# mhamilton723/STEGO

Measured on NVIDIA H100. Metric: train-step images/sec, higher is better.
Workload: dtype bf16

## Files before the change

include/stego_b200.h:

```cpp
#ifndef STEGO_B200_H_
#define STEGO_B200_H_

#ifdef __cplusplus
extern "C" {
#endif

#define STEGO_API

STEGO_API int stego_version(void);
STEGO_API const char* stego_last_error(void);
STEGO_API long long stego_launch_count(void);

STEGO_API int stego_gemm_bf16(const void* A, int lda, int a_mn_major, const void* B, int ldb, int b_mn_major,
                              int M, int N, int K, void* out, int ldo, int out_bf16, const float* bias, int act,
                              const float* residual, int ldr, int row_div, int splits, int atomic_out,
                              void* stream);

STEGO_API int stego_gemm_bf16_batched(const void* A, int lda, long long a_batch_stride, int a_mn_major, const void* B,
                                      int ldb, long long b_batch_stride, int b_mn_major, int batch, int M, int N, int K,
                                      void* out, int ldo, long long out_batch_stride, int out_bf16, const float* bias,
                                      int act, void* stream);

STEGO_API int stego_vit_patchify(const float* img, void* out_bf16, int B, int H, int W, int patch, void* stream);
STEGO_API int stego_vit_patchify_bf16(const void* img_bf16, void* out_bf16, int B, int H, int W, int patch,
                                      void* stream);
STEGO_API int stego_vit_patchify_tta(const void* img, int img_is_bf16, void* out_bf16, int B, int H, int W, int patch,
                                     void* stream);
STEGO_API int stego_vit_cls_rows(float* x, const float* cls_token, const float* pos_embed, int B, int ntok, int E,
                                 void* stream);
STEGO_API int stego_layernorm_bf16(const float* x, const float* gamma, const float* beta, void* out_bf16, int rows,
                                   int E, float eps, int drop_cls_ntok, void* stream);
STEGO_API int stego_layernorm_gap(const float* x, const float* gamma, const float* beta, float* out, int B, int ntok,
                                  int E, float eps, void* stream);
STEGO_API int stego_linear_rows_f32(const float* x, const void* w_bf16, int ldw, const float* bias, float* out, int B,
                                    int N, int K, void* stream);
STEGO_API int stego_attention_fwd(const void* qkv, void* out, int B, int N, int E, int heads, void* stream);
STEGO_API int stego_attention_probs(const void* qkv, float* probs, int B, int N, int E, int heads, void* stream);

STEGO_API int stego_sample_norm_fwd(const void* src, const void* src_pos, int src_is_bf16, long long stride_b,
                                    long long stride_c, long long stride_y, long long stride_x,
                                    const float* chan_scale, const float* chan_scale_pos, const float* coords1,
                                    const float* coords2, const long long* perms, void* tiles, int B, int C,
                                    int Cpad, int H, int W, int feature_samples, int nslots, int perms_are_raw_randperm,
                                    void* stream);
STEGO_API int stego_sample_labels_fwd(const void* label, const void* label_pos, int label_bytes, const float* coords1,
                                      const float* coords2, const long long* perms, void* tiles, int B, int n_classes,
                                      int Cpad, int H, int W, int feature_samples, int nslots,
                                      int perms_are_raw_randperm, void* stream);
STEGO_API int stego_corr_loss_fwd(const void* feat_tiles, const void* code_tiles, int B, int feature_samples, int E,
                                  int D, int nslots, int ncalls, const int* slot_of_call_host,
                                  const float* shifts_host, int pointwise, int zero_clamp, int stabilize,
                                  float* partials, float* stats, float* cd_out, float* fdc_out, float* loss_out,
                                  void* stream);
STEGO_API int stego_corr_loss_bwd(const void* feat_tiles, const void* code_tiles, int B, int feature_samples, int E,
                                  int D, int nslots, int ncalls, const int* slot_of_call_host,
                                  const float* shifts_host, int pointwise, int zero_clamp, int stabilize,
                                  const float* stats, const float* gscale, const float* gelem, const float* gcd,
                                  float* dtiles, void* stream);
STEGO_API int stego_sample_norm_bwd(const float* code, const float* code_pos, long long stride_b, long long stride_c,
                                    long long stride_y, long long stride_x, const float* coords1,
                                    const float* coords2, const long long* perms, const float* dtiles, float* dcode,
                                    float* dcode_pos, int B, int C, int H, int W, int feature_samples, int nslots,
                                    int perms_are_raw_randperm, void* stream);

STEGO_API int stego_corr_loss_tiled_fwd(const void* feat_tiles, const void* code_tiles, int B, int feature_samples,
                                        int E, int D, int nslots, int ncalls, const int* slot_of_call_host,
                                        const float* shifts_host, int pointwise, int zero_clamp, int stabilize,
                                        float* row_partials, float* row_means, float* stats, float* cd_out,
                                        float* fdc_out, float* loss_out, void* stream);
STEGO_API int stego_corr_loss_tiled_bwd(const void* feat_tiles, const void* code_tiles, int B, int feature_samples,
                                        int E, int D, int nslots, int ncalls, const int* slot_of_call_host,
                                        const float* shifts_host, int pointwise, int zero_clamp, int stabilize,
                                        const float* stats, const float* row_means, const float* gscale,
                                        const float* gelem, const float* gcd, float* dtiles, void* stream);

STEGO_API int stego_salience_counts(const void* salience, const void* salience_pos, int mask_bytes, int B, int H, int W,
                                    int* counts, void* stream);
STEGO_API int stego_salience_coords(const void* salience, const void* salience_pos, int mask_bytes, int B, int H, int W,
                                    int feature_samples, long long seed, const long long* offsets,
                                    const void* draws_u32, const float* u_reg1, const float* u_reg2,
                                    const float* u_keep, float* coords1, float* coords2, void* scratch, void* stream);
STEGO_API long long stego_salience_scratch_bytes(int B, int H, int W);

STEGO_API int stego_aug_record_words(void);
STEGO_API long long stego_aug_scratch_bytes(int B, int size);
STEGO_API int stego_aug_views(const float* img, long long stride_b, long long stride_c, long long stride_y,
                              long long stride_x, int B, int H, int W, int size, const int* records, void* scratch,
                              float* img_aug, float* coord_aug, void* stream);

STEGO_API int stego_tb_tables(double* edges, float* thresholds);
STEGO_API int stego_tb_histogram(const float* values, long long n, const float* thresholds, long long* counts,
                                 double* cta_partials, double* stats, void* stream);
STEGO_API int stego_corr_loss_fwd_hist(const void* feat_tiles, const void* code_tiles, int B, int feature_samples,
                                       int E, int D, int nslots, int ncalls, const int* slot_of_call_host,
                                       const float* shifts_host, int pointwise, int zero_clamp, int stabilize,
                                       float* partials, float* stats, float* cd_out, float* fdc_out, float* loss_out,
                                       const float* thresholds, long long* hist_counts, double* hist_cta_partials,
                                       double* hist_stats, void* stream);
STEGO_API int stego_corr_loss_tiled_fwd_hist(const void* feat_tiles, const void* code_tiles, int B,
// ... 189 lines not shown
```

stego_b200/csrc/attention.cu:

```cuda
#include <stdlib.h>

#include "common.cuh"
#include "host_util.h"

namespace stego {

constexpr int ATT_BQ = 128;
constexpr int ATT_BKV = 64;
constexpr int ATT_D = 64;
constexpr int ATT_STAGES = 4;
constexpr int ATT_THREADS = 288;

constexpr uint32_t ATT_Q_BYTES = 128 * 64 * 2;
constexpr uint32_t ATT_KV_BYTES = 64 * 64 * 2;
constexpr uint32_t ATT_SMEM_Q = 0;
constexpr uint32_t ATT_SMEM_KV = ATT_Q_BYTES;
constexpr uint32_t ATT_SMEM_BAR = ATT_SMEM_KV + ATT_STAGES * 2 * ATT_KV_BYTES;
constexpr uint32_t ATT_SMEM_TOTAL = ATT_SMEM_BAR + 128;

struct AttnParams {
  int N;
  int E;
  float scale_log2e;
};

__global__ void __launch_bounds__(ATT_THREADS, 2)
attention_fwd_kernel(const __grid_constant__ CUtensorMap tmQKV, const __grid_constant__ CUtensorMap tmOut, AttnParams p) {
  extern __shared__ __align__(1024) uint8_t smem[];
  if ((smem_u32(smem) & 1023u) != 0u) __trap();
  uint64_t* bars = reinterpret_cast<uint64_t*>(smem + ATT_SMEM_BAR);
  uint64_t* q_full = bars;
  uint64_t* kv_full = bars + 1;
  uint64_t* kv_empty = kv_full + ATT_STAGES;

  const int warp = threadIdx.x >> 5;
  const int lane = threadIdx.x & 31;
  const int q0 = blockIdx.x * ATT_BQ;
  const int head = blockIdx.y;
  const int img = blockIdx.z;
  const int nkv = (p.N + ATT_BKV - 1) / ATT_BKV;

  if (threadIdx.x == 0) {
    mbar_init(q_full, 1);
    for (int s = 0; s < ATT_STAGES; ++s) {
      mbar_init(&kv_full[s], 1);
      mbar_init(&kv_empty[s], 2);
    }
    fence_barrier_init();
  }
  __syncthreads();

  if (warp == 8) {
    if (lane == 0) {
      tma_prefetch_desc(&tmQKV);
      tma_prefetch_desc(&tmOut);
      mbar_arrive_expect_tx(q_full, ATT_Q_BYTES);
      tma_load_3d(smem + ATT_SMEM_Q, &tmQKV, q_full, head * ATT_D, q0, img);
      tma_load_3d(smem + ATT_SMEM_Q + ATT_Q_BYTES / 2, &tmQKV, q_full, head * ATT_D, q0 + 64, img);
      uint32_t stage = 0, phase = 0;
      for (int j = 0; j < nkv; ++j) {
        mbar_wait(&kv_empty[stage], phase ^ 1u);
        uint8_t* sk = smem + ATT_SMEM_KV + stage * 2 * ATT_KV_BYTES;
        mbar_arrive_expect_tx(&kv_full[stage], 2 * ATT_KV_BYTES);
        tma_load_3d(sk, &tmQKV, &kv_full[stage], p.E + head * ATT_D, j * ATT_BKV, img);
        tma_load_3d(sk + ATT_KV_BYTES, &tmQKV, &kv_full[stage], 2 * p.E + head * ATT_D, j * ATT_BKV, img);
        if (++stage == ATT_STAGES) { stage = 0; phase ^= 1u; }
      }
    }
    return;
  }

  const int wg = warp >> 2;
  const int wq = warp & 3;
  const bool leader = (threadIdx.x & 127) == 0;
  const float c = p.scale_log2e;
  constexpr uint32_t DESC_HI = smem_desc_hi_sw128(1024);
  uint8_t* sq = smem + ATT_SMEM_Q + wg * (ATT_Q_BYTES / 2);
  const uint32_t q_lo = smem_desc_lo(smem_u32(sq), 16);
  const uint32_t k_lo0 = smem_desc_lo(smem_u32(smem + ATT_SMEM_KV), 16);
  const uint32_t v_lo0 = smem_desc_lo(smem_u32(smem + ATT_SMEM_KV + ATT_KV_BYTES), 8192);
  float o[32];
#pragma unroll
  for (int i = 0; i < 32; ++i) o[i] = 0.f;
  float m_run[2] = {-INFINITY, -INFINITY}, l_run[2] = {0.f, 0.f};
  mbar_wait(q_full, 0);
  uint32_t stage = 0, phase = 0;
  for (int j = 0; j < nkv; ++j) {
    mbar_wait(&kv_full[stage], phase);
    const uint32_t k_lo = k_lo0 + stage * ((2 * ATT_KV_BYTES) >> 4);
    const uint32_t v_lo = v_lo0 + stage * ((2 * ATT_KV_BYTES) >> 4);
    float s[32];
    wgmma_fence();
#pragma unroll
    for (uint32_t k = 0; k < ATT_D / 16; ++k)
      wgmma_ss<64, 0, 0>(s, smem_desc_join(q_lo + k * 2, DESC_HI), smem_desc_join(k_lo + k * 2, DESC_HI), k > 0 ? 1u : 0u);
    wgmma_commit();
    wgmma_wait<0>();
    fence_operands(s);
    const int valid = p.N - j * ATT_BKV;
    if (valid < ATT_BKV) {
#pragma unroll
      for (int i = 0; i < 32; ++i)
        if (8 * (i >> 2) + 2 * (lane & 3) + (i & 1) >= valid) s[i] = -INFINITY;
    }
    float alpha[2], mc[2];
#pragma unroll
    for (int h = 0; h < 2; ++h) {
      float mx = -INFINITY;
#pragma unroll
      for (int i = 0; i < 8; ++i) mx = fmaxf(mx, fmaxf(s[4 * i + 2 * h], s[4 * i + 2 * h + 1]));
      mx = fmaxf(mx, __shfl_xor_sync(0xffffffffu, mx, 1));
      mx = fmaxf(mx, __shfl_xor_sync(0xffffffffu, mx, 2));
      const float m_new = fmaxf(m_run[h], mx);
      alpha[h] = ex2_approx((m_run[h] - m_new) * c);
      m_run[h] = m_new;
      mc[h] = m_new * c;
    }
    uint32_t a[4][4];
    float rs[2] = {0.f, 0.f};
#pragma unroll
    for (int i = 0; i < 8; ++i) {
#pragma unroll
// ... 244 lines not shown
```

stego_b200/csrc/gemm.cu:

```cuda
#include <stdlib.h>
#include <string.h>

#include "common.cuh"
#include "epilogue.cuh"
#include "host_util.h"

namespace stego {

constexpr int GEMM_BM = 128;
constexpr int GEMM_BN = 128;
constexpr int GEMM_BK = 64;
constexpr int GEMM_THREADS = 384;
constexpr uint32_t GEMM_STAGE_BYTES = (GEMM_BM + GEMM_BN) * GEMM_BK * 2;
constexpr uint32_t GEMM_CHUNK_BYTES = GEMM_BM * 128;

struct GemmParams {
  int M, N, K;
  int splits;
  int kb_per_split;
  void* out;
  int ldo;
  int out_bf16;
  const float* bias;
  int act;
  const float* residual;
  int ldr;
  int row_div;
  int atomic;
  int vec_ok;
  int reduce_add;
  int batch;
  long long out_bs;
  long long res_bs;
};

template <int BN>
__device__ __forceinline__ void gemm_bias_act(float (&acc)[BN / 2], const GemmParams& p, int col_base) {
  if (p.bias != nullptr) {
#pragma unroll
    for (int c = 0; c < BN / 8; ++c) {
      const int col = col_base + 8 * c;
      float b0 = 0.f, b1 = 0.f;
      if (col + 1 < p.N && p.vec_ok) {
        const float2 b2 = __ldg(reinterpret_cast<const float2*>(p.bias + col));
        b0 = b2.x; b1 = b2.y;
      } else {
        if (col < p.N) b0 = __ldg(p.bias + col);
        if (col + 1 < p.N) b1 = __ldg(p.bias + col + 1);
      }
      acc[4 * c + 0] += b0; acc[4 * c + 1] += b1;
      acc[4 * c + 2] += b0; acc[4 * c + 3] += b1;
    }
  }
  if (p.act == 1) {
    if (p.out_bf16) {
#pragma unroll
      for (int j = 0; j < BN / 2; j += 8) gelu_erf_poly8(acc + j);
    } else {
#pragma unroll
      for (int j = 0; j < BN / 2; ++j) acc[j] = gelu_erf(acc[j]);
    }
  } else if (p.act == 2) {
#pragma unroll
    for (int j = 0; j < BN / 2; ++j) acc[j] = fmaxf(acc[j], 0.0f);
  }
}

template <int BN>
__device__ __forceinline__ void gemm_store_regs(const float (&acc)[BN / 2], const GemmParams& p, int row_top,
                                                int col_base, int tb) {
  void* const outp = p.out_bf16 ? static_cast<void*>(reinterpret_cast<bf16*>(p.out) + tb * p.out_bs)
                                : static_cast<void*>(reinterpret_cast<float*>(p.out) + tb * p.out_bs);
  const float* const resp = p.residual ? p.residual + tb * p.res_bs : nullptr;
#pragma unroll
  for (int h = 0; h < 2; ++h) {
    const int row = row_top + 8 * h;
    if (row >= p.M) continue;
    int out_row = row, res_row = row;
    if (p.row_div > 0) {
      out_row = row + row / p.row_div + 1;
      res_row = row % p.row_div + 1;
    }
    const size_t obase = static_cast<size_t>(out_row) * p.ldo;
    const size_t rbase = static_cast<size_t>(res_row) * p.ldr;
#pragma unroll
    for (int c = 0; c < BN / 8; ++c) {
      const int col = col_base + 8 * c;
      if (col >= p.N) break;
      const bool two = col + 1 < p.N;
      float x0 = acc[4 * c + 2 * h], x1 = acc[4 * c + 2 * h + 1];
      if (p.atomic) {
        float* o = reinterpret_cast<float*>(outp) + obase + col;
        atomicAdd(o, x0);
        if (two) atomicAdd(o + 1, x1);
        continue;
      }
      const bool vec = two && p.vec_ok;
      if (resp != nullptr) {
        if (vec) {
          const float2 r = *reinterpret_cast<const float2*>(resp + rbase + col);
          x0 += r.x; x1 += r.y;
        } else {
          x0 += resp[rbase + col];
          if (two) x1 += resp[rbase + col + 1];
        }
      }
      if (p.out_bf16) {
        bf16* o = reinterpret_cast<bf16*>(outp) + obase + col;
        if (vec) {
          *reinterpret_cast<uint32_t*>(o) = pack_bf16x2(x0, x1);
        } else {
          o[0] = __float2bfloat16_rn(x0);
          if (two) o[1] = __float2bfloat16_rn(x1);
        }
      } else {
        float* o = reinterpret_cast<float*>(outp) + obase + col;
// ... 27 lines not shown
    for (int h = 0; h < 2; ++h) {
#pragma unroll
      for (int e2 = 0; e2 < 2; ++e2) {
        const uint32_t rp = rbase + (64 * h + 8 * e2) * 128u;
        if constexpr (kBf16) {
#pragma unroll
          for (int j = 0; j < 8; ++j) {
            const int c = 8 * ch + j;
            st_shared_b32(rp + (((uint32_t)j ^ swz) << 4) + 4 * q,
                          pack_bf16x2(acc[h][4 * c + 2 * e2], acc[h][4 * c + 2 * e2 + 1]));
          }
        } else {
#pragma unroll
          for (int j = 0; j < 4; ++j) {
            const int c = 4 * ch + j;
            const uint32_t unit = 2 * j + (q >> 1);
            st_shared_v2_f32(rp + ((unit ^ swz) << 4) + 8 * (q & 1), acc[h][4 * c + 2 * e2],
                             acc[h][4 * c + 2 * e2 + 1]);
          }
        }
      }
    }
    fence_proxy_async_smem();
    named_bar_sync(bar_id, 128);
    if (issuer) {
      const int col = n0 + ch * kCols;
      if (p.reduce_add) tma_reduce_add_3d(buf, tm_out, col, m0, tb);
      else tma_store_3d(buf, tm_out, col, m0, tb);
      tma_commit_group();
    }
  }
}

template <int kStages>
__device__ __forceinline__ void ring_advance(uint32_t& stage, uint32_t& phase, int n) {
  stage += n;
  while (stage >= kStages) { stage -= kStages; phase ^= 1u; }
}

template <int kStages, bool A_MN, bool B_MN, bool kTmaEpi>
__global__ void __launch_bounds__(GEMM_THREADS, 1)
gemm_bf16_kernel(const __grid_constant__ CUtensorMap tmA, const __grid_constant__ CUtensorMap tmB,
                 const __grid_constant__ CUtensorMap tmOut, GemmParams p) {
  constexpr uint32_t A_BYTES = GEMM_BM * GEMM_BK * 2;
  constexpr uint32_t STAGE_BYTES = GEMM_STAGE_BYTES;

  extern __shared__ __align__(1024) uint8_t smem_raw[];
  uint8_t* smem = reinterpret_cast<uint8_t*>((reinterpret_cast<uintptr_t>(smem_raw) + 1023) & ~uintptr_t(1023));
  uint8_t* staging = smem + kStages * STAGE_BYTES;
  uint64_t* full_bar = reinterpret_cast<uint64_t*>(staging + (kTmaEpi ? 4 * GEMM_CHUNK_BYTES : 0));
  uint64_t* empty_bar = full_bar + kStages;
  uint64_t* turn_bar = empty_bar + kStages;

  const int warp = threadIdx.x >> 5;
  const int lane = threadIdx.x & 31;
  const int wg = warp >> 2;

  const int tiles_m = (p.M + GEMM_BM - 1) / GEMM_BM;
  const int tiles_n = (p.N + GEMM_BN - 1) / GEMM_BN;
  const int num_kb = (p.K + GEMM_BK - 1) / GEMM_BK;
  const int tiles_per_batch = tiles_m * tiles_n * p.splits;
  const int total_tiles = tiles_per_batch * p.batch;
  const int sched_start = static_cast<int>(blockIdx.x);
  const int sched_step = static_cast<int>(gridDim.x);

  if (threadIdx.x == 0) {
    tma_prefetch_desc(&tmA);
    tma_prefetch_desc(&tmB);
    if (kTmaEpi) tma_prefetch_desc(&tmOut);
    for (int s = 0; s < kStages; ++s) {
      mbar_init(&full_bar[s], 1);
      mbar_init(&empty_bar[s], 1);
    }
    mbar_init(&turn_bar[0], 1);
    mbar_init(&turn_bar[1], 1);
    fence_barrier_init();
  }
  __syncthreads();

  if (wg == 0) {
    warpgroup_reg_dealloc<40>();
    if (threadIdx.x == 0) {
      uint32_t stage = 0, phase = 0;
      for (int t = sched_start; t < total_tiles; t += sched_step) {
        const int tb = t / tiles_per_batch, tl = t % tiles_per_batch;
        const int split = tl % p.splits;
        const int tn = (tl / p.splits) % tiles_n;
        const int tm = tl / (p.splits * tiles_n);
        const int kb0 = split * p.kb_per_split;
        const int kb1 = min(num_kb, kb0 + p.kb_per_split);
        for (int kb = kb0; kb < kb1; ++kb) {
          mbar_wait(&empty_bar[stage], phase ^ 1u);
          uint8_t* sa = smem + stage * STAGE_BYTES;
          uint8_t* sb = sa + A_BYTES;
          mbar_arrive_expect_tx(&full_bar[stage], STAGE_BYTES);
          if (!A_MN) {
            tma_load_3d(sa, &tmA, &full_bar[stage], kb * GEMM_BK, tm * GEMM_BM, tb);
          } else {
#pragma unroll
            for (int blk = 0; blk < GEMM_BM / 64; ++blk)
              tma_load_3d(sa + blk * 8192, &tmA, &full_bar[stage], tm * GEMM_BM + blk * 64, kb * GEMM_BK, tb);
          }
          if (!B_MN) {
            tma_load_3d(sb, &tmB, &full_bar[stage], kb * GEMM_BK, tn * GEMM_BN, tb);
          } else {
#pragma unroll
            for (int blk = 0; blk < GEMM_BN / 64; ++blk)
              tma_load_3d(sb + blk * 8192, &tmB, &full_bar[stage], tn * GEMM_BN + blk * 64, kb * GEMM_BK, tb);
          }
          if (++stage == kStages) { stage = 0; phase ^= 1u; }
        }
      }
    }
  } else {
    warpgroup_reg_alloc<232>();
    const int mwg = wg - 1;
    constexpr uint32_t DESC_HI = smem_desc_hi_sw128(1024);
    constexpr uint32_t A_KSTEP = A_MN ? (2048u >> 4) : (32u >> 4);
    constexpr uint32_t B_KSTEP = B_MN ? (2048u >> 4) : (32u >> 4);
    constexpr uint32_t A_HALF = 8192u >> 4;
    const uint32_t a_lo0 = smem_desc_lo(smem_u32(smem), 8192u);
    const uint32_t b_lo0 = smem_desc_lo(smem_u32(smem) + A_BYTES, 8192u);
    const bool leader = (threadIdx.x & 127) == 0;
    const int wq = (threadIdx.x >> 5) & 3;
    uint32_t stage = 0, phase = 0;
    float acc[2][GEMM_BN / 2];
    int i = 0;
    for (int t = sched_start; t < total_tiles; t += sched_step, ++i) {
      const int tb = t / tiles_per_batch, tl = t % tiles_per_batch;
      const int split = tl % p.splits;
      const int tn = (tl / p.splits) % tiles_n;
      const int tm = tl / (p.splits * tiles_n);
      const int kb0 = split * p.kb_per_split;
      const int kb1 = min(num_kb, kb0 + p.kb_per_split);
      if ((i & 1) != mwg) {
        ring_advance<kStages>(stage, phase, kb1 - kb0);
        continue;
      }
      if (i > 0) mbar_wait(&turn_bar[mwg], ((i - 1) >> 1) & 1);
#pragma unroll
      for (int j = 0; j < GEMM_BN / 2; ++j) { acc[0][j] = 0.f; acc[1][j] = 0.f; }
      uint32_t prev_stage = 0;
      for (int kb = kb0; kb < kb1; ++kb) {
        mbar_wait(&full_bar[stage], phase);
        const uint32_t a_lo = a_lo0 + stage * (STAGE_BYTES >> 4);
        const uint32_t b_lo = b_lo0 + stage * (STAGE_BYTES >> 4);
        fence_operands(acc[0]);
        fence_operands(acc[1]);
        wgmma_fence();
#pragma unroll
        for (uint32_t k = 0; k < GEMM_BK / 16; ++k) {
          const uint64_t db = smem_desc_join(b_lo + k * B_KSTEP, DESC_HI);
#pragma unroll
          for (uint32_t h = 0; h < 2; ++h)
            wgmma_ss<GEMM_BN, A_MN ? 1 : 0, B_MN ? 1 : 0>(
                acc[h], smem_desc_join(a_lo + h * A_HALF + k * A_KSTEP, DESC_HI), db, 1u);
        }
        wgmma_commit();
        wgmma_wait<1>();
        if (kb > kb0 && leader) mbar_arrive(&empty_bar[prev_stage]);
        prev_stage = stage;
        if (++stage == kStages) { stage = 0; phase ^= 1u; }
      }
      if (leader) mbar_arrive(&turn_bar[mwg ^ 1]);
      wgmma_wait<0>();
      fence_operands(acc[0]);
      fence_operands(acc[1]);
      if (kb1 > kb0 && leader) mbar_arrive(&empty_bar[prev_stage]);
      const int col_base = tn * GEMM_BN + 2 * (lane & 3);
      gemm_bias_act<GEMM_BN>(acc[0], p, col_base);
      gemm_bias_act<GEMM_BN>(acc[1], p, col_base);
      if constexpr (kTmaEpi) {
        const uint32_t st = smem_u32(staging) + mwg * 2 * GEMM_CHUNK_BYTES;
        if (p.out_bf16) gemm_store_tma<true>(acc, p, &tmOut, st, 1 + mwg, leader, tm * GEMM_BM, tn * GEMM_BN, tb);
        else gemm_store_tma<false>(acc, p, &tmOut, st, 1 + mwg, leader, tm * GEMM_BM, tn * GEMM_BN, tb);
      } else {
        const int row_top = tm * GEMM_BM + wq * 16 + (lane >> 2);
        gemm_store_regs<GEMM_BN>(acc[0], p, row_top, col_base, tb);
        gemm_store_regs<GEMM_BN>(acc[1], p, row_top + 64, col_base, tb);
      }
    }
    if (kTmaEpi && leader) tma_wait_group<0>();
  }
}

template <int kStages, bool A_MN, bool B_MN, bool kTmaEpi>
static int launch_gemm(const CUtensorMap& tmA, const CUtensorMap& tmB, const CUtensorMap& tmOut, const GemmParams& p,
                       cudaStream_t stream) {
  constexpr size_t smem = size_t(kStages) * GEMM_STAGE_BYTES + (kTmaEpi ? 4 * GEMM_CHUNK_BYTES : 0) + 1024 + 256;
  static_assert(smem <= 232448, "exceeds the 227 KB of shared memory a CTA can opt into");
  constexpr auto kern = gemm_bf16_kernel<kStages, A_MN, B_MN, kTmaEpi>;
  if (const int rc = opt_in_smem<kern>(smem, "gemm_bf16_kernel"); rc != STEGO_OK) return rc;
  const int tiles_m = (p.M + GEMM_BM - 1) / GEMM_BM;
  const int tiles_n = (p.N + GEMM_BN - 1) / GEMM_BN;
  const int tiles = tiles_m * tiles_n * p.splits * p.batch;
  const int grid = tiles < num_sms() ? tiles : num_sms();
  kern<<<grid, GEMM_THREADS, smem, stream>>>(tmA, tmB, tmOut, p);
  STEGO_CHECK_LAUNCH("gemm_bf16_kernel launch");
  return STEGO_OK;
}

template <bool A_MN, bool B_MN>
static int launch_gemm_epi(bool tma_epi, const CUtensorMap& tmA, const CUtensorMap& tmB, const CUtensorMap& tmOut,
                           const GemmParams& p, cudaStream_t stream) {
  if (tma_epi) return launch_gemm<5, A_MN, B_MN, true>(tmA, tmB, tmOut, p, stream);
  return launch_gemm<6, A_MN, B_MN, false>(tmA, tmB, tmOut, p, stream);
}

}

using namespace stego;

static int gemm_impl(const void* A, int lda, long long a_bs, int a_mn_major, const void* B, int ldb, long long b_bs,
                     int b_mn_major, int batch, int M, int N, int K, void* out, int ldo, long long out_bs, int out_bf16,
                     const float* bias, int act, const float* residual, int ldr, long long res_bs, int row_div, int splits,
                     int atomic_out, cudaStream_t stream) {
  STEGO_CHECK_ARG(A && B && out, "stego_gemm_bf16: null pointer");
  STEGO_CHECK_ARG(M > 0 && N > 0 && K > 0 && batch > 0, "stego_gemm_bf16: bad sizes M=%d N=%d K=%d batch=%d", M, N, K, batch);
  STEGO_CHECK_ARG(lda % 8 == 0 && ldb % 8 == 0, "stego_gemm_bf16: lda/ldb must be multiples of 8 elements");
  STEGO_CHECK_ARG(batch == 1 || (a_bs % 8 == 0 && b_bs % 8 == 0 && row_div == 0),
                  "stego_gemm_bf16_batched: operand batch strides must be multiples of 8 elements");
  STEGO_CHECK_ARG(act >= 0 && act <= 2, "stego_gemm_bf16: act=%d", act);
  STEGO_CHECK_ARG(!(atomic_out && out_bf16), "stego_gemm_bf16: atomic output must be fp32");
  STEGO_CHECK_ARG(splits >= 1, "stego_gemm_bf16: splits=%d", splits);
  STEGO_CHECK_ARG(splits == 1 || atomic_out, "stego_gemm_bf16: split-K requires atomic_out");
  STEGO_CHECK_ARG(!atomic_out || (bias == nullptr && act == 0 && residual == nullptr),
                  "stego_gemm_bf16: atomic_out takes no bias, act or residual (bias=%p act=%d residual=%p)",
                  (const void*)bias, act, (const void*)residual);
  STEGO_CHECK_ARG(lda >= (a_mn_major ? M : K) && ldb >= (b_mn_major ? N : K),
                  "stego_gemm_bf16: lda=%d / ldb=%d shorter than a row (M=%d N=%d K=%d, a_mn_major=%d b_mn_major=%d)",
                  lda, ldb, M, N, K, a_mn_major, b_mn_major);
  STEGO_CHECK_ARG(ldo >= N && (residual == nullptr || ldr >= N),
                  "stego_gemm_bf16: ldo=%d / ldr=%d shorter than a row of N=%d", ldo, ldr, N);
  if (batch == 1) {
    a_bs = static_cast<long long>(a_mn_major ? K : M) * lda;
    b_bs = static_cast<long long>(b_mn_major ? K : N) * ldb;
    out_bs = static_cast<long long>(M) * ldo;
    res_bs = 0;
  }

  GemmParams p;
  p.M = M; p.N = N; p.K = K;
  const int num_kb = (K + GEMM_BK - 1) / GEMM_BK;
  if (splits > num_kb) splits = num_kb;
  p.kb_per_split = (num_kb + splits - 1) / splits;
  p.splits = (num_kb + p.kb_per_split - 1) / p.kb_per_split;
  p.out = out; p.ldo = ldo; p.out_bf16 = out_bf16;
  p.bias = bias; p.act = act;
  p.residual = residual; p.ldr = ldr;
  p.row_div = row_div; p.atomic = atomic_out;
  p.batch = batch; p.out_bs = out_bs; p.res_bs = res_bs;
  const size_t esz = out_bf16 ? 2 : 4;
  const size_t pair = 2 * esz;
  p.vec_ok = ((reinterpret_cast<uintptr_t>(out) % pair) == 0) && (ldo % 2 == 0) && (out_bs % 2 == 0) &&
             (residual == nullptr || ((reinterpret_cast<uintptr_t>(residual) % 8) == 0 && ldr % 2 == 0 && res_bs % 2 == 0)) &&
             (bias == nullptr || (reinterpret_cast<uintptr_t>(bias) % 8) == 0);
  const bool in_place = residual != nullptr && residual == out && ldr == ldo && !out_bf16;
  const bool tma_epi = !atomic_out && row_div == 0 && (residual == nullptr || in_place) &&
                       (reinterpret_cast<uintptr_t>(out) % 16) == 0 && (static_cast<size_t>(ldo) * esz) % 16 == 0 &&
                       (static_cast<size_t>(out_bs) * esz) % 16 == 0 && (static_cast<size_t>(N) * esz) % 16 == 0;
  p.reduce_add = tma_epi && in_place;

  CUtensorMap tmA, tmB, tmOut;
  int rc;
  {
    uint64_t dims[3] = {a_mn_major ? (uint64_t)M : (uint64_t)K, a_mn_major ? (uint64_t)K : (uint64_t)M, (uint64_t)batch};
    uint64_t str[2] = {(uint64_t)lda * 2, (uint64_t)a_bs * 2};
    uint32_t box[3] = {64, a_mn_major ? 64u : (uint32_t)GEMM_BM, 1};
    if ((rc = make_tmap_bf16(&tmA, A, 3, dims, str, box)) != STEGO_OK) return rc;
  }
  {
    uint64_t dims[3] = {b_mn_major ? (uint64_t)N : (uint64_t)K, b_mn_major ? (uint64_t)K : (uint64_t)N, (uint64_t)batch};
    uint64_t str[2] = {(uint64_t)ldb * 2, (uint64_t)b_bs * 2};
    uint32_t box[3] = {64, b_mn_major ? 64u : (uint32_t)GEMM_BN, 1};
    if ((rc = make_tmap_bf16(&tmB, B, 3, dims, str, box)) != STEGO_OK) return rc;
  }
  if (tma_epi) {
    uint64_t dims[3] = {(uint64_t)N, (uint64_t)M, (uint64_t)batch};
    uint64_t str[2] = {(uint64_t)ldo * esz, (uint64_t)out_bs * esz};
    uint32_t box[3] = {(uint32_t)(128 / esz), (uint32_t)GEMM_BM, 1};
    rc = out_bf16 ? make_tmap_bf16(&tmOut, out, 3, dims, str, box) : make_tmap_f32(&tmOut, out, 3, dims, str, box);
    if (rc != STEGO_OK) return rc;
  } else {
    memset(&tmOut, 0, sizeof(tmOut));
  }
  if (!a_mn_major && !b_mn_major) return launch_gemm_epi<false, false>(tma_epi, tmA, tmB, tmOut, p, stream);
  if (!a_mn_major && b_mn_major) return launch_gemm_epi<false, true>(tma_epi, tmA, tmB, tmOut, p, stream);
  if (a_mn_major && b_mn_major) return launch_gemm_epi<true, true>(tma_epi, tmA, tmB, tmOut, p, stream);
  return launch_gemm_epi<true, false>(tma_epi, tmA, tmB, tmOut, p, stream);
}

extern "C" int stego_gemm_bf16(const void* A, int lda, int a_mn_major, const void* B, int ldb, int b_mn_major, int M,
                               int N, int K, void* out, int ldo, int out_bf16, const float* bias, int act,
                               const float* residual, int ldr, int row_div, int splits, int atomic_out,
                               void* stream_) {
  return gemm_impl(A, lda, 0, a_mn_major, B, ldb, 0, b_mn_major, 1, M, N, K, out, ldo, 0, out_bf16, bias, act, residual, ldr, 0,
                   row_div, splits, atomic_out, reinterpret_cast<cudaStream_t>(stream_));
}

extern "C" int stego_gemm_bf16_batched(const void* A, int lda, long long a_batch_stride, int a_mn_major, const void* B,
                                       int ldb, long long b_batch_stride, int b_mn_major, int batch, int M, int N, int K,
                                       void* out, int ldo, long long out_batch_stride, int out_bf16, const float* bias,
                                       int act, void* stream_) {
  return gemm_impl(A, lda, a_batch_stride, a_mn_major, B, ldb, b_batch_stride, b_mn_major, batch, M, N, K, out, ldo,
                   out_batch_stride, out_bf16, bias, act, nullptr, 0, 0, 0, 1, 0, reinterpret_cast<cudaStream_t>(stream_));
}
```

stego_b200/csrc/vit_misc.cu:

```cuda
#include "common.cuh"
#include "host_util.h"

namespace stego {

__device__ __forceinline__ uint32_t swap_bf16x2(uint32_t v) { return __byte_perm(v, 0, 0x1032); }

template <int P, typename T, bool MIRROR>
__global__ void patchify_kernel(const T* __restrict__ img, bf16* __restrict__ out, int B, int H, int W) {
  const int fh = H / P, fw = W / P;
  const long long total = 1ll * (MIRROR ? 2 * B : B) * fh * fw * 3 * P;
  const long long idx = 1ll * blockIdx.x * blockDim.x + threadIdx.x;
  if (idx >= total) return;
  const int ky = idx % P;
  const int c = (idx / P) % 3;
  const long long patch = idx / (3 * P);
  const int px = patch % fw;
  const int py = (patch / fw) % fh;
  const int b = patch / (1ll * fw * fh);
  const bool flip = MIRROR && b >= B;
  const int sb = flip ? b - B : b, sx = flip ? fw - 1 - px : px;
  const T* src = img + ((1ll * sb * 3 + c) * H + (py * P + ky)) * W + sx * P;
  bf16* dst = out + patch * (3 * P * P) + c * P * P + ky * P;
  static_assert(P == 8 || P == 16, "patch size");
#pragma unroll
  for (int v = 0; v < P / 8; ++v) {
    const int sv = flip ? P / 8 - 1 - v : v;
    uint4 w;
    if constexpr (sizeof(T) == 2) {
      w = *reinterpret_cast<const uint4*>(src + sv * 8);
    } else {
      const float4 a = *reinterpret_cast<const float4*>(src + sv * 8);
      const float4 b4 = *reinterpret_cast<const float4*>(src + sv * 8 + 4);
      w.x = pack_bf16x2(a.x, a.y);
      w.y = pack_bf16x2(a.z, a.w);
      w.z = pack_bf16x2(b4.x, b4.y);
      w.w = pack_bf16x2(b4.z, b4.w);
    }
    if (flip) w = make_uint4(swap_bf16x2(w.w), swap_bf16x2(w.z), swap_bf16x2(w.y), swap_bf16x2(w.x));
    *reinterpret_cast<uint4*>(dst + v * 8) = w;
  }
}

__global__ void cls_rows_kernel(float* __restrict__ x, const float* __restrict__ cls, const float* __restrict__ pos,
                                int B, int ntok, int E) {
  const int i = blockIdx.x * blockDim.x + threadIdx.x;
  if (i >= B * E) return;
  const int b = i / E, e = i % E;
  x[(1ll * b * ntok) * E + e] = cls[e] + pos[e];
}

template <int V4>
__global__ void __launch_bounds__(256)
layernorm_kernel(const float* __restrict__ x, const float* __restrict__ gamma, const float* __restrict__ beta,
                 bf16* __restrict__ out, int rows, float eps, int drop_cls) {
  constexpr int E = V4 * 128;
  const int row = blockIdx.x * (blockDim.x >> 5) + (threadIdx.x >> 5);
  if (row >= rows) return;
  const int lane = threadIdx.x & 31;
  long long orow = row;
  if (drop_cls > 0) {
    const int t = row % drop_cls;
    if (t == 0) return;
    orow = 1ll * (row / drop_cls) * (drop_cls - 1) + (t - 1);
  }
  const float4* xr = reinterpret_cast<const float4*>(x + 1ll * row * E);
  float4 v[V4];
  float s = 0.f;
#pragma unroll
  for (int i = 0; i < V4; ++i) {
    v[i] = xr[lane + 32 * i];
    s += (v[i].x + v[i].y) + (v[i].z + v[i].w);
  }
  const float mean = __fmul_rn(warp_sum(s), 1.0f / E);
  float q = 0.f;
#pragma unroll
  for (int i = 0; i < V4; ++i) {
    const float a = v[i].x - mean, b = v[i].y - mean, c = v[i].z - mean, d = v[i].w - mean;
    q += (a * a + b * b) + (c * c + d * d);
  }
  const float rstd = rsqrtf(warp_sum(q) * (1.0f / E) + eps);
  const float4* g4 = reinterpret_cast<const float4*>(gamma);
  const float4* b4 = reinterpret_cast<const float4*>(beta);
  uint2* o = reinterpret_cast<uint2*>(out + orow * E);
#pragma unroll
  for (int i = 0; i < V4; ++i) {
    const float4 g = __ldg(g4 + lane + 32 * i);
    const float4 bb = __ldg(b4 + lane + 32 * i);
    uint2 w;
    w.x = pack_bf16x2((v[i].x - mean) * rstd * g.x + bb.x, (v[i].y - mean) * rstd * g.y + bb.y);
    w.y = pack_bf16x2((v[i].z - mean) * rstd * g.z + bb.z, (v[i].w - mean) * rstd * g.w + bb.w);
    o[lane + 32 * i] = w;
  }
}

template <int V4>
__global__ void __launch_bounds__(256)
layernorm_gap_kernel(const float* __restrict__ x, const float* __restrict__ gamma, const float* __restrict__ beta,
                     float* __restrict__ out, int ntok, float eps, int rows_per_cta) {
  constexpr int E = V4 * 128;
  __shared__ float4 red[8][V4 * 32];
  const int b = blockIdx.y;
  const int warp = threadIdx.x >> 5, lane = threadIdx.x & 31;
  const int t0 = 1 + blockIdx.x * rows_per_cta;
  const int t1 = min(ntok, t0 + rows_per_cta);
  const float4* g4 = reinterpret_cast<const float4*>(gamma);
  float4 g[V4], acc[V4];
#pragma unroll
  for (int i = 0; i < V4; ++i) {
    g[i] = __ldg(g4 + lane + 32 * i);
    acc[i] = make_float4(0.f, 0.f, 0.f, 0.f);
  }
  int nrows = 0;
  for (int t = t0 + warp; t < t1; t += 8) {
    const float4* xr = reinterpret_cast<const float4*>(x + (1ll * b * ntok + t) * E);
    float4 v[V4];
    float s = 0.f;
#pragma unroll
    for (int i = 0; i < V4; ++i) {
      v[i] = xr[lane + 32 * i];
      s += (v[i].x + v[i].y) + (v[i].z + v[i].w);
    }
    const float mean = __fmul_rn(warp_sum(s), 1.0f / E);
    float q = 0.f;
#pragma unroll
    for (int i = 0; i < V4; ++i) {
      const float a = v[i].x - mean, bq = v[i].y - mean, c = v[i].z - mean, d = v[i].w - mean;
      q += (a * a + bq * bq) + (c * c + d * d);
    }
    const float rstd = rsqrtf(warp_sum(q) * (1.0f / E) + eps);
#pragma unroll
    for (int i = 0; i < V4; ++i) {
      acc[i].x += (v[i].x - mean) * rstd * g[i].x;
      acc[i].y += (v[i].y - mean) * rstd * g[i].y;
      acc[i].z += (v[i].z - mean) * rstd * g[i].z;
      acc[i].w += (v[i].w - mean) * rstd * g[i].w;
    }
    ++nrows;
  }
#pragma unroll
  for (int i = 0; i < V4; ++i) red[warp][lane + 32 * i] = acc[i];
// ... 160 lines not shown
```

stego_b200/dino/vision_transformer.py:

```python
from __future__ import annotations

import math
import threading
from functools import partial
from typing import Dict, List, Optional, Tuple

import torch
import torch.nn as nn

from .. import ops

_PREPARE_LOCK = threading.RLock()


def _to_device(w, dev):
    if isinstance(w, dict):
        return {k: _to_device(v, dev) for k, v in w.items()}
    if isinstance(w, list):
        return [_to_device(v, dev) for v in w]
    return w.to(dev) if isinstance(w, torch.Tensor) else w


class Mlp(nn.Module):

# ... 122 lines not shown
                proj_b=f32(blk.attn.proj.bias, E),
                n2w=f32(blk.norm2.weight, E), n2b=f32(blk.norm2.bias, E), eps2=blk.norm2.eps,
                fc1_w=blk.mlp.fc1.weight.detach().to(torch.bfloat16).contiguous(), fc1_b=f32(blk.mlp.fc1.bias, blk.mlp.fc1.out_features),
                fc2_w=blk.mlp.fc2.weight.detach().to(torch.bfloat16).contiguous(), fc2_b=f32(blk.mlp.fc2.bias, E)))
        w["blocks"] = blocks
        w["nw"] = self.norm.weight.detach().float().contiguous()
        w["nb"] = self.norm.bias.detach().float().contiguous()
        return w

    def interpolate_pos_encoding(self, x, w, h):
        npatch = x.shape[1] - 1
        N = self.pos_embed.shape[1] - 1
        if npatch == N and w == h:
            return self.pos_embed
        dim = x.shape[-1]
        p = self.patch_embed.patch_size
        w0, h0 = w // p + 0.1, h // p + 0.1
        side = int(math.sqrt(N))
        grid = self.pos_embed[:, 1:].reshape(1, side, side, dim).permute(0, 3, 1, 2)
        grid = nn.functional.interpolate(grid, scale_factor=(w0 / math.sqrt(N), h0 / math.sqrt(N)), mode='bicubic')
        assert int(w0) == grid.shape[-2] and int(h0) == grid.shape[-1]
        grid = grid.permute(0, 2, 3, 1).reshape(1, -1, dim)
        return torch.cat((self.pos_embed[:, :1], grid), dim=1)

    def _pos_for(self, H: int, W: int, device=None) -> torch.Tensor:
        master = self._root()
        home = master.cls_token.device
        dev = home if device is None else torch.device(device)
        self._prepared(dev)
        with _PREPARE_LOCK:
            cache = master._cache["pos"]
            if (H, W, home) not in cache:
                p = master.patch_embed.patch_size
                ntok = (H // p) * (W // p) + 1
                with torch.no_grad():
                    dummy = torch.empty(1, ntok, master.embed_dim, device="meta")
                    pos = master.interpolate_pos_encoding(dummy, H, W)
                cache[(H, W, home)] = pos.detach().float().reshape(ntok, master.embed_dim).contiguous()
            if (H, W, dev) not in cache:
                cache[(H, W, dev)] = cache[(H, W, home)].to(dev)
            return cache[(H, W, dev)]

    @torch.no_grad()
    def forward_tokens(self, img: torch.Tensor, want_qkv: bool = False, taps: Optional["BlockTaps"] = None,
                       stop_before_last: bool = False, mirror: bool = False
                       ) -> Tuple[torch.Tensor, Optional[torch.Tensor]]:
        if not img.is_cuda:
            raise RuntimeError("stego_b200: the DINO ViT forward only exists as sm_90a kernels (no CPU fallback)")
        w = self._prepared(img.device)
        img = (img if img.dtype == torch.bfloat16 else img.float()).contiguous()
        B, _, H, W = img.shape
        B = 2 * B if mirror else B
        p = self.patch_embed.patch_size
        E, heads = self.embed_dim, self.num_heads
        hw = (H // p) * (W // p)
        N = hw + 1
        dev = img.device
        pos = self._pos_for(H, W, dev)
        rows = ops.patchify_tta(img, p) if mirror else ops.patchify(img, p)
        x = torch.empty(B * N, E, dtype=torch.float32, device=dev)
        ops.gemm(rows, w["pe_w"], x, M=B * hw, N=E, K=3 * p * p, bias=w["pe_b"], residual=pos, row_div=hw)
        ops.cls_rows(x, w["cls"], pos, B, N)
        y = torch.empty(B * N, E, dtype=torch.bfloat16, device=dev)
        qkv = torch.empty(B * N, 3 * E, dtype=torch.bfloat16, device=dev)
        ao = torch.empty(B * N, E, dtype=torch.bfloat16, device=dev)
        hid = torch.empty(B * N, w["blocks"][0]["fc1_w"].shape[0], dtype=torch.bfloat16, device=dev)
        Hd = hid.shape[1]
        blocks = w["blocks"]
        depth = len(blocks)
        for i, bw in enumerate(blocks[:-1] if stop_before_last else blocks):
            tap = taps is not None and depth - i <= taps.n
            ops.layernorm(x, bw["n1w"], bw["n1b"], y, eps=bw["eps1"])
            ops.gemm(y, bw["qkv_w"], qkv, M=B * N, N=3 * E, K=E, bias=bw["qkv_b"])
            if tap:
                taps.qkv.append(qkv.clone())
                if taps.probs:
                    taps.attn.append(ops.attention_probs(
                        qkv, torch.empty(B, heads, N, N, dtype=torch.float32, device=dev), B, N, E, heads))
                if taps.stop_at_last_probs and i == depth - 1:
                    break
            ops.attention(qkv, ao, B, N, E, heads)
            ops.gemm(ao, bw["proj_w"], x, M=B * N, N=E, K=E, bias=bw["proj_b"], residual=x)
            ops.layernorm(x, bw["n2w"], bw["n2b"], y, eps=bw["eps2"])
            ops.gemm(y, bw["fc1_w"], hid, M=B * N, N=Hd, K=E, bias=bw["fc1_b"], act=ops.ACT_GELU)
            ops.gemm(hid, bw["fc2_w"], x, M=B * N, N=E, K=Hd, bias=bw["fc2_b"], residual=x)
            if tap:
                taps.x.append(x.clone())
        return x, (qkv if want_qkv else None)

    @torch.no_grad()
    def patch_features(self, img: torch.Tensor, use_graph: bool = False, mirror: bool = False) -> torch.Tensor:
        return self._tokens(img, use_graph, "feat", mirror)

    @torch.no_grad()
    def key_features(self, img: torch.Tensor, use_graph: bool = False, mirror: bool = False) -> torch.Tensor:
        return self._tokens(img, use_graph, "KK", mirror)

    def _tokens(self, img, use_graph: bool, kind: str, mirror: bool = False) -> torch.Tensor:
        kind = kind + "+mirror" if mirror else kind
        if use_graph and (img[0] if isinstance(img, (list, tuple)) else img).is_cuda:
            return self._graphed(img, kind)
        if isinstance(img, (list, tuple)):
            img = torch.cat(list(img), 0)
        return self._eager(img, kind)

    def _eager(self, img: torch.Tensor, kind: str) -> torch.Tensor:
        mirror = kind.endswith("+mirror")
        if kind.startswith("feat"):
            return self._patch_features_eager(img, mirror)
        return self._key_features_eager(img, mirror)

    def _graphed(self, img, kind: str) -> torch.Tensor:
        from .. import _lib
        parts = list(img) if isinstance(img, (list, tuple)) else [img]
        self._prepared(parts[0].device)
        graphs = self._root()._cache.setdefault("graphs", {})
        shape = (sum(p.shape[0] for p in parts),) + tuple(parts[0].shape[1:])
        dt = torch.bfloat16 if all(p.dtype == torch.bfloat16 for p in parts) else torch.float32
        key = (kind, shape, parts[0].device.index, dt)
        if key not in graphs:
            img = torch.cat([p.to(dt) for p in parts], 0) if len(parts) > 1 else parts[0].to(dt)
            self._eager(img, kind)
            static_in = img.detach().contiguous().clone()
            with torch.cuda.device(static_in.device):
                graphs[key] = (_lib.Graph(lambda: self._eager(static_in, kind)), static_in)
        g, static_in = graphs[key]
        off = 0
        for part in parts:
            if part.data_ptr() != static_in[off].data_ptr():
                static_in[off:off + part.shape[0]].copy_(part)
            off += part.shape[0]
        g.replay()
        return g.result

    def graph_input(self, kind: str, shape, device, dtype=torch.float32):
        return self._root()._cache.get("graphs", {}).get((kind, tuple(shape), device.index, dtype), (None, None))[1]

    def _patch_features_eager(self, img: torch.Tensor, mirror: bool = False) -> torch.Tensor:
        B = img.shape[0] * (2 if mirror else 1)
        x, _ = self.forward_tokens(img, mirror=mirror)
        w = self._prepared(x.device)
        N = x.shape[0] // B
        out = torch.empty(B * (N - 1), self.embed_dim, dtype=torch.bfloat16, device=x.device)
        ops.layernorm(x, w["nw"], w["nb"], out, eps=self.norm.eps, drop_cls_ntok=N)
        return out.view(B, N - 1, self.embed_dim)

    def _key_features_eager(self, img: torch.Tensor, mirror: bool = False) -> torch.Tensor:
        B, E = img.shape[0] * (2 if mirror else 1), self.embed_dim
        x, _ = self.forward_tokens(img, stop_before_last=True, mirror=mirror)
        bw = self._prepared(x.device)["blocks"][-1]
        N = x.shape[0] // B
        y = torch.empty(B * (N - 1), E, dtype=torch.bfloat16, device=x.device)
        ops.layernorm(x, bw["n1w"], bw["n1b"], y, eps=bw["eps1"], drop_cls_ntok=N)
        out = torch.empty(B * (N - 1), E, dtype=torch.bfloat16, device=x.device)
        ops.gemm(y, bw["qkv_w"][E:2 * E], out, M=B * (N - 1), N=E, K=E, bias=bw["qkv_b"][E:2 * E])
        return out.view(B, N - 1, E)

    @torch.no_grad()
    def pooled_patch_features(self, img: torch.Tensor) -> torch.Tensor:
        from .. import _lib
        B = img.shape[0]
        x, _ = self.forward_tokens(img)
        w = self._prepared(x.device)
        out = torch.zeros(B, self.embed_dim, dtype=torch.float32, device=x.device)
        _lib.check(_lib.load().stego_layernorm_gap(_lib.ptr(x), _lib.ptr(w["nw"]), _lib.ptr(w["nb"]), _lib.ptr(out), B,
                                                   x.shape[0] // B, self.embed_dim, float(self.norm.eps), _lib.stream()),
                   "stego_layernorm_gap")
# ... 82 lines not shown
```

stego_b200/ops.py:

```python
from __future__ import annotations

from typing import Optional

import torch

from . import _lib

ACT_NONE, ACT_GELU, ACT_RELU = 0, 1, 2


def gemm(a: torch.Tensor, b: torch.Tensor, out: torch.Tensor, *, M: int, N: int, K: int,
         a_mn: bool = False, b_mn: bool = False, bias: Optional[torch.Tensor] = None, act: int = ACT_NONE,
         residual: Optional[torch.Tensor] = None, row_div: int = 0, splits: int = 1,
         atomic: bool = False) -> torch.Tensor:
    _lib.require_cuda(a, b, out, bias, residual)
    assert a.dtype == torch.bfloat16 and b.dtype == torch.bfloat16
    assert a.dim() == 2 and b.dim() == 2 and out.dim() == 2
    assert a.stride(1) == 1 and b.stride(1) == 1 and out.stride(1) == 1
    assert out.dtype in (torch.bfloat16, torch.float32)
    if bias is not None:
        assert bias.dtype == torch.float32 and bias.is_contiguous()
    if residual is not None:
        assert residual.dtype == torch.float32 and residual.stride(1) == 1
    rc = _lib.load().stego_gemm_bf16(
        _lib.ptr(a), a.stride(0), int(a_mn), _lib.ptr(b), b.stride(0), int(b_mn), M, N, K,
        _lib.ptr(out), out.stride(0), int(out.dtype == torch.bfloat16), _lib.ptr(bias), act,
        _lib.ptr(residual), residual.stride(0) if residual is not None else 0, row_div, splits, int(atomic),
        _lib.stream())
    _lib.check(rc, "stego_gemm_bf16")
    return out


def wgrad_splits(K: int, out_rows: int, out_cols: int, num_sms: int) -> int:
    tiles = ((out_rows + 127) // 128) * ((out_cols + 127) // 128)
    return max(1, min(K // 512, num_sms // tiles))


def gemm_batched(a: torch.Tensor, b: torch.Tensor, out: torch.Tensor, *, a_mn: bool = False, b_mn: bool = False,
                 bias: Optional[torch.Tensor] = None, act: int = ACT_NONE) -> torch.Tensor:
    _lib.require_cuda(a, b, out, bias)
    assert a.dtype == torch.bfloat16 and b.dtype == torch.bfloat16 and a.dim() == 3 and b.dim() == 3 and out.dim() == 3
    assert a.stride(2) == 1 and b.stride(2) == 1 and out.stride(2) == 1 and out.dtype in (torch.bfloat16, torch.float32)
    n = a.shape[0]
    M, K = (a.shape[2], a.shape[1]) if a_mn else (a.shape[1], a.shape[2])
    N = b.shape[2] if b_mn else b.shape[1]
    assert b.shape[0] == n and out.shape == (n, M, N) and (b.shape[1] if b_mn else b.shape[2]) == K
    rc = _lib.load().stego_gemm_bf16_batched(
        _lib.ptr(a), a.stride(1), a.stride(0), int(a_mn), _lib.ptr(b), b.stride(1), b.stride(0), int(b_mn), n, M, N, K,
        _lib.ptr(out), out.stride(1), out.stride(0), int(out.dtype == torch.bfloat16), _lib.ptr(bias), act, _lib.stream())
    _lib.check(rc, "stego_gemm_bf16_batched")
    return out


def patchify(img: torch.Tensor, patch: int) -> torch.Tensor:
    _lib.require_cuda(img)
    assert img.dtype in (torch.float32, torch.bfloat16) and img.is_contiguous() and img.shape[1] == 3
    B, _, H, W = img.shape
    out = torch.empty(B * (H // patch) * (W // patch), 3 * patch * patch, dtype=torch.bfloat16, device=img.device)
    lib = _lib.load()
    fn = lib.stego_vit_patchify if img.dtype == torch.float32 else lib.stego_vit_patchify_bf16
    _lib.check(fn(_lib.ptr(img), _lib.ptr(out), B, H, W, patch, _lib.stream()), "stego_vit_patchify")
    return out


def patchify_tta(img: torch.Tensor, patch: int) -> torch.Tensor:
    _lib.require_cuda(img)
    assert img.dtype in (torch.float32, torch.bfloat16) and img.is_contiguous() and img.shape[1] == 3
    B, _, H, W = img.shape
    out = torch.empty(2 * B * (H // patch) * (W // patch), 3 * patch * patch, dtype=torch.bfloat16, device=img.device)
    _lib.check(_lib.load().stego_vit_patchify_tta(_lib.ptr(img), int(img.dtype == torch.bfloat16), _lib.ptr(out), B, H, W,
                                                  patch, _lib.stream()), "stego_vit_patchify_tta")
    return out


def cls_rows(x: torch.Tensor, cls_token: torch.Tensor, pos_embed: torch.Tensor, B: int, ntok: int) -> None:
    E = x.shape[-1]
    _lib.check(_lib.load().stego_vit_cls_rows(_lib.ptr(x), _lib.ptr(cls_token), _lib.ptr(pos_embed), B, ntok, E,
                                              _lib.stream()), "stego_vit_cls_rows")


def layernorm(x: torch.Tensor, gamma: torch.Tensor, beta: torch.Tensor, out: torch.Tensor, eps: float = 1e-6,
              drop_cls_ntok: int = 0) -> torch.Tensor:
    _lib.require_cuda(x, gamma, beta, out)
    assert x.dtype == torch.float32 and x.is_contiguous() and out.dtype == torch.bfloat16 and out.is_contiguous()
    rows, E = x.shape
    _lib.check(_lib.load().stego_layernorm_bf16(_lib.ptr(x), _lib.ptr(gamma), _lib.ptr(beta), _lib.ptr(out), rows, E,
                                                eps, drop_cls_ntok, _lib.stream()), "stego_layernorm_bf16")
    return out


def linear_rows_f32(x: torch.Tensor, w: torch.Tensor, bias: Optional[torch.Tensor] = None) -> torch.Tensor:
    _lib.require_cuda(x, w, bias)
    assert x.dtype == torch.float32 and x.dim() == 2 and x.is_contiguous()
    assert w.dtype == torch.bfloat16 and w.dim() == 2 and w.stride(1) == 1 and w.shape[1] == x.shape[1]
    if bias is not None:
        assert bias.dtype == torch.float32 and bias.is_contiguous() and bias.numel() == w.shape[0]
    B, K = x.shape
    N = w.shape[0]
    out = torch.empty(B, N, dtype=torch.float32, device=x.device)
    _lib.check(_lib.load().stego_linear_rows_f32(_lib.ptr(x), _lib.ptr(w), w.stride(0), _lib.ptr(bias), _lib.ptr(out),
                                                 B, N, K, _lib.stream()), "stego_linear_rows_f32")
    return out


def attention(qkv: torch.Tensor, out: torch.Tensor, B: int, N: int, E: int, heads: int) -> torch.Tensor:
    _lib.require_cuda(qkv, out)
    assert qkv.dtype == torch.bfloat16 and qkv.is_contiguous() and out.dtype == torch.bfloat16 and out.is_contiguous()
# ... 38 lines not shown
```

Measured before the change: 3017.

## Alternate tile traversal direction across consecutive kernels for L2 reuse

Reverses the processing order in the attention kernel (images), the layernorm kernel (rows), and the fc1 GEMM (tiles, via a new descending entry point). Each consumer then starts on the data its producer wrote last, which is more likely to still be in L2. The GEMM adds a runtime flag and one extra index computation per tile. It may also shift how work is balanced across SMs.

```diff
diff --git a/include/stego_b200.h b/include/stego_b200.h
--- a/include/stego_b200.h
+++ b/include/stego_b200.h
@@ -15,6 +15,11 @@
                               int M, int N, int K, void* out, int ldo, int out_bf16, const float* bias, int act,
                               const float* residual, int ldr, int row_div, int splits, int atomic_out,
                               void* stream);
+
+STEGO_API int stego_gemm_bf16_desc(const void* A, int lda, int a_mn_major, const void* B, int ldb, int b_mn_major,
+                                   int M, int N, int K, void* out, int ldo, int out_bf16, const float* bias, int act,
+                                   const float* residual, int ldr, int row_div, int splits, int atomic_out,
+                                   void* stream);
 
 STEGO_API int stego_gemm_bf16_batched(const void* A, int lda, long long a_batch_stride, int a_mn_major, const void* B,
                                       int ldb, long long b_batch_stride, int b_mn_major, int batch, int M, int N, int K,
diff --git a/stego_b200/csrc/attention.cu b/stego_b200/csrc/attention.cu
--- a/stego_b200/csrc/attention.cu
+++ b/stego_b200/csrc/attention.cu
@@ -37,7 +37,7 @@
   const int lane = threadIdx.x & 31;
   const int q0 = blockIdx.x * ATT_BQ;
   const int head = blockIdx.y;
-  const int img = blockIdx.z;
+  const int img = gridDim.z - 1 - blockIdx.z;
   const int nkv = (p.N + ATT_BKV - 1) / ATT_BKV;
 
   if (threadIdx.x == 0) {
diff --git a/stego_b200/csrc/gemm.cu b/stego_b200/csrc/gemm.cu
--- a/stego_b200/csrc/gemm.cu
+++ b/stego_b200/csrc/gemm.cu
@@ -32,6 +32,7 @@
   int batch;
   long long out_bs;
   long long res_bs;
+  int descending;
 };
 
 template <int BN>
@@ -225,7 +226,8 @@
     warpgroup_reg_dealloc<40>();
     if (threadIdx.x == 0) {
       uint32_t stage = 0, phase = 0;
-      for (int t = sched_start; t < total_tiles; t += sched_step) {
+      for (int ts = sched_start; ts < total_tiles; ts += sched_step) {
+        const int t = p.descending ? total_tiles - 1 - ts : ts;
         const int tb = t / tiles_per_batch, tl = t % tiles_per_batch;
         const int split = tl % p.splits;
         const int tn = (tl / p.splits) % tiles_n;
@@ -269,7 +271,8 @@
     uint32_t stage = 0, phase = 0;
     float acc[2][GEMM_BN / 2];
     int i = 0;
-    for (int t = sched_start; t < total_tiles; t += sched_step, ++i) {
+    for (int ts = sched_start; ts < total_tiles; ts += sched_step, ++i) {
+      const int t = p.descending ? total_tiles - 1 - ts : ts;
       const int tb = t / tiles_per_batch, tl = t % tiles_per_batch;
       const int split = tl % p.splits;
       const int tn = (tl / p.splits) % tiles_n;
@@ -357,7 +360,7 @@
 static int gemm_impl(const void* A, int lda, long long a_bs, int a_mn_major, const void* B, int ldb, long long b_bs,
                      int b_mn_major, int batch, int M, int N, int K, void* out, int ldo, long long out_bs, int out_bf16,
                      const float* bias, int act, const float* residual, int ldr, long long res_bs, int row_div, int splits,
-                     int atomic_out, cudaStream_t stream) {
+                     int atomic_out, int descending, cudaStream_t stream) {
   STEGO_CHECK_ARG(A && B && out, "stego_gemm_bf16: null pointer");
   STEGO_CHECK_ARG(M > 0 && N > 0 && K > 0 && batch > 0, "stego_gemm_bf16: bad sizes M=%d N=%d K=%d batch=%d", M, N, K, batch);
   STEGO_CHECK_ARG(lda % 8 == 0 && ldb % 8 == 0, "stego_gemm_bf16: lda/ldb must be multiples of 8 elements");
@@ -393,6 +396,7 @@
   p.residual = residual; p.ldr = ldr;
   p.row_div = row_div; p.atomic = atomic_out;
   p.batch = batch; p.out_bs = out_bs; p.res_bs = res_bs;
+  p.descending = descending;
   const size_t esz = out_bf16 ? 2 : 4;
   const size_t pair = 2 * esz;
   p.vec_ok = ((reinterpret_cast<uintptr_t>(out) % pair) == 0) && (ldo % 2 == 0) && (out_bs % 2 == 0) &&
@@ -438,7 +442,15 @@
                                const float* residual, int ldr, int row_div, int splits, int atomic_out,
                                void* stream_) {
   return gemm_impl(A, lda, 0, a_mn_major, B, ldb, 0, b_mn_major, 1, M, N, K, out, ldo, 0, out_bf16, bias, act, residual, ldr, 0,
-                   row_div, splits, atomic_out, reinterpret_cast<cudaStream_t>(stream_));
+                   row_div, splits, atomic_out, 0, reinterpret_cast<cudaStream_t>(stream_));
+}
+
+extern "C" int stego_gemm_bf16_desc(const void* A, int lda, int a_mn_major, const void* B, int ldb, int b_mn_major,
+                                    int M, int N, int K, void* out, int ldo, int out_bf16, const float* bias, int act,
+                                    const float* residual, int ldr, int row_div, int splits, int atomic_out,
+                                    void* stream_) {
+  return gemm_impl(A, lda, 0, a_mn_major, B, ldb, 0, b_mn_major, 1, M, N, K, out, ldo, 0, out_bf16, bias, act, residual, ldr, 0,
+                   row_div, splits, atomic_out, 1, reinterpret_cast<cudaStream_t>(stream_));
 }
 
 extern "C" int stego_gemm_bf16_batched(const void* A, int lda, long long a_batch_stride, int a_mn_major, const void* B,
@@ -446,5 +458,6 @@
                                        void* out, int ldo, long long out_batch_stride, int out_bf16, const float* bias,
                                        int act, void* stream_) {
   return gemm_impl(A, lda, a_batch_stride, a_mn_major, B, ldb, b_batch_stride, b_mn_major, batch, M, N, K, out, ldo,
-                   out_batch_stride, out_bf16, bias, act, nullptr, 0, 0, 0, 1, 0, reinterpret_cast<cudaStream_t>(stream_));
-}
+                   out_batch_stride, out_bf16, bias, act, nullptr, 0, 0, 0, 1, 0, 0,
+                   reinterpret_cast<cudaStream_t>(stream_));
+}
diff --git a/stego_b200/csrc/vit_misc.cu b/stego_b200/csrc/vit_misc.cu
--- a/stego_b200/csrc/vit_misc.cu
+++ b/stego_b200/csrc/vit_misc.cu
@@ -54,8 +54,9 @@
 layernorm_kernel(const float* __restrict__ x, const float* __restrict__ gamma, const float* __restrict__ beta,
                  bf16* __restrict__ out, int rows, float eps, int drop_cls) {
   constexpr int E = V4 * 128;
-  const int row = blockIdx.x * (blockDim.x >> 5) + (threadIdx.x >> 5);
-  if (row >= rows) return;
+  const int r = blockIdx.x * (blockDim.x >> 5) + (threadIdx.x >> 5);
+  if (r >= rows) return;
+  const int row = rows - 1 - r;
   const int lane = threadIdx.x & 31;
   long long orow = row;
   if (drop_cls > 0) {
diff --git a/stego_b200/dino/vision_transformer.py b/stego_b200/dino/vision_transformer.py
--- a/stego_b200/dino/vision_transformer.py
+++ b/stego_b200/dino/vision_transformer.py
@@ -228,7 +228,7 @@
             ops.attention(qkv, ao, B, N, E, heads)
             ops.gemm(ao, bw["proj_w"], x, M=B * N, N=E, K=E, bias=bw["proj_b"], residual=x)
             ops.layernorm(x, bw["n2w"], bw["n2b"], y, eps=bw["eps2"])
-            ops.gemm(y, bw["fc1_w"], hid, M=B * N, N=Hd, K=E, bias=bw["fc1_b"], act=ops.ACT_GELU)
+            ops.gemm(y, bw["fc1_w"], hid, M=B * N, N=Hd, K=E, bias=bw["fc1_b"], act=ops.ACT_GELU, descending=True)
             ops.gemm(hid, bw["fc2_w"], x, M=B * N, N=E, K=Hd, bias=bw["fc2_b"], residual=x)
             if tap:
                 taps.x.append(x.clone())
diff --git a/stego_b200/ops.py b/stego_b200/ops.py
--- a/stego_b200/ops.py
+++ b/stego_b200/ops.py
@@ -12,7 +12,7 @@
 def gemm(a: torch.Tensor, b: torch.Tensor, out: torch.Tensor, *, M: int, N: int, K: int,
          a_mn: bool = False, b_mn: bool = False, bias: Optional[torch.Tensor] = None, act: int = ACT_NONE,
          residual: Optional[torch.Tensor] = None, row_div: int = 0, splits: int = 1,
-         atomic: bool = False) -> torch.Tensor:
+         atomic: bool = False, descending: bool = False) -> torch.Tensor:
     _lib.require_cuda(a, b, out, bias, residual)
     assert a.dtype == torch.bfloat16 and b.dtype == torch.bfloat16
     assert a.dim() == 2 and b.dim() == 2 and out.dim() == 2
@@ -22,7 +22,8 @@
         assert bias.dtype == torch.float32 and bias.is_contiguous()
     if residual is not None:
         assert residual.dtype == torch.float32 and residual.stride(1) == 1
-    rc = _lib.load().stego_gemm_bf16(
+    lib = _lib.load()
+    rc = (lib.stego_gemm_bf16_desc if descending else lib.stego_gemm_bf16)(
         _lib.ptr(a), a.stride(0), int(a_mn), _lib.ptr(b), b.stride(0), int(b_mn), M, N, K,
         _lib.ptr(out), out.stride(0), int(out.dtype == torch.bfloat16), _lib.ptr(bias), act,
         _lib.ptr(residual), residual.stride(0) if residual is not None else 0, row_div, splits, int(atomic),
```

New measurement: 3051, median of 6. +1.2%, better.
